# zju-pi/diff-sampler

Hardware: AMD Instinct MI355X
Metric: images/sec (whole node) at NFE=10, EDM CIFAR-10 (higher is better)
Workload: dtype fp32; 1 GPU; EDM CIFAR-10 32x32 SongUNet (55.7M params), DPM-Solver++(2M) logSNR NFE=10, batch 256/GPU; launch=eager

## Files before the change

diff_sampler_amd/csrc/conv3x3_wino.hip:

```cpp
#include <type_traits>

#include "igemm_common.h"

namespace igemm {
namespace {

typedef float f32x2 __attribute__((ext_vector_type(2)));

constexpr int WV_NO_NORM = 2, WV_NO_HALO = 4, WV_NO_DMA = 8, WV_NO_EPI = 16;
constexpr int WINO_K = 8;
constexpr int WINO_POS = 2 * 64 * 4;
constexpr int WINO_IMG = 16 * WINO_POS;
constexpr int WINO_NSH = 4;
constexpr int WINO_EPI_LD = 36;

#define DS_WINO_WAIT_VM0() do { __builtin_amdgcn_s_waitcnt(0x0F70); asm volatile("" ::: "memory"); } while (0)
#define DS_WINO_WAIT_VM(n) do { __builtin_amdgcn_s_waitcnt(0x0F70 | (n)); asm volatile("" ::: "memory"); } while (0)

template <int VAR, int NORM, int NSL>
__global__ void __launch_bounds__(256, 1) conv3x3_wino_kernel(const KParams p) {
    extern __shared__ __attribute__((aligned(16))) float smem[];
    float* Us = smem;
    float* Vs = smem + 2 * WINO_IMG;
    float* Hs = smem + 4 * WINO_IMG;

    const int tid = threadIdx.x, lane = tid & 63;
    const int wave = __builtin_amdgcn_readfirstlane(tid >> 6);
    const int wr = wave >> 1, wc = wave & 1;
    int mt, nt;
    if (!decode_tile(blockIdx.x, p.mtiles, p.ntiles, mt, nt)) return;
    const int m0 = mt * 256, n0 = nt * 64;
    const int img0 = m0 / p.HW;
    const int r0 = (m0 - img0 * p.HW) / p.W;
    const int WPH = p.WP >> 1, Wt = p.W >> 1;
    const int Ctot = p.c0 + p.c1;
    const int nslabs = Ctot / WINO_K;
    constexpr bool kDma = !(VAR & WV_NO_DMA), kHalo = !(VAR & WV_NO_HALO);
    constexpr int kNorm = (VAR & WV_NO_NORM) ? 0 : NORM;

    const int kh_h = tid & 1;
    const int h_buf = p.NP * WINO_K + 4;
    unsigned h_off0[WINO_NSH], h_off1[WINO_NSH];
    int h_lds[WINO_NSH];
#pragma unroll
    for (int j = 0; j < WINO_NSH; ++j) {
        const int hp = (tid + j * 256) >> 1;
        const int hr = hp / p.WP, hc = hp - hr * p.WP;
        const int y = r0 + hr - 1, x = hc - 1;
        const bool in = hp < p.NP;
        const bool ok = in && (unsigned)y < (unsigned)p.H && (unsigned)x < (unsigned)p.W;
        const int pix = min(max(y, 0), p.H - 1) * p.W + min(max(x, 0), p.W - 1);
        h_off0[j] = (unsigned)(pix * p.lda0 + kh_h * 4) * 4u;
        h_off1[j] = (unsigned)(pix * p.lda1 + kh_h * 4) * 4u;
        const int cell = (((kh_h * 2 + (hc & 1)) * p.HP + hr) * WPH + (hc >> 1)) * 4;
        h_lds[j] = ok ? cell : p.NP * WINO_K;
        if (in && !ok) {
            const f32x4 z = {0.f, 0.f, 0.f, 0.f};
            *reinterpret_cast<f32x4*>(Hs + cell) = z;
            *reinterpret_cast<f32x4*>(Hs + h_buf + cell) = z;
        }
    }
    const float* a0i = p.a0 + (size_t)img0 * p.HW * p.lda0;
    const float* a1i = p.a1 + (size_t)img0 * p.HW * p.lda1;
    const float* cpi = p.norm + (size_t)img0 * 3 * Ctot;
    unsigned c_lane = (unsigned)(kh_h * 16);
    struct HaloRegs {
        f32x4 h[WINO_NSH];
        f32x4 mu = {0.f, 0.f, 0.f, 0.f}, ga = {1.f, 1.f, 1.f, 1.f}, be = {0.f, 0.f, 0.f, 0.f};
    };
    HaloRegs hreg;
    float h_t[4 * WINO_NSH], h_u[4 * WINO_NSH];
    const float* h_src = nullptr;
    unsigned h_sel = 0;
    auto halo_src = [&](int s) {
        const int c = s * WINO_K;
        const bool first = c < p.c0;
        h_src = first ? a0i + c : a1i + (c - p.c0);
        h_sel = (unsigned)__builtin_amdgcn_readfirstlane(first ? -1 : 0);
        asm volatile("" : "+s"(h_sel));
    };
    auto halo_load1 = [&](HaloRegs& R, auto J) {
        constexpr int j = decltype(J)::value;
        if constexpr (j >= NSL) return;
        const unsigned off = (h_off0[j] & h_sel) | (h_off1[j] & ~h_sel);
        R.h[j] = *reinterpret_cast<const f32x4*>(reinterpret_cast<const char*>(h_src) + off);
    };
    auto coef_load1 = [&](HaloRegs& R, int s, auto I) {
        constexpr int i = decltype(I)::value;
        if constexpr (NORM != 0) {
            const char* cs = reinterpret_cast<const char*>(cpi + (size_t)i * Ctot + s * WINO_K);
            asm volatile("" : "+v"(c_lane));
            const f32x4 v = *reinterpret_cast<const f32x4*>(cs + c_lane);
            if constexpr (i == 0) R.mu = v; else if constexpr (i == 1) R.ga = v; else R.be = v;
        }
    };
    auto halo_chain = [&](HaloRegs& R, float* hs, auto C, auto ST) {
        constexpr int c = decltype(C)::value, st = decltype(ST)::value, j = c >> 2, e = c & 3;
        if constexpr (j >= NSL) return;
        if constexpr (st == 0 && kNorm != 0) {
            h_t[c] = __builtin_fmaf(R.h[j][e] - R.mu[e], R.ga[e], R.be[e]);
            if constexpr (kNorm == 2) h_u[c] = __expf(-h_t[c]);
        }
        if constexpr (st == 1 && kNorm == 2) h_u[c] = __builtin_amdgcn_rcpf(1.0f + h_u[c]);
        if constexpr (st == 2) {
            float v = R.h[j][e];
            if constexpr (kNorm == 1) v = h_t[c];
            if constexpr (kNorm == 2) v = h_t[c] * h_u[c];
            R.h[j][e] = v;
            if constexpr (e == 3) *reinterpret_cast<f32x4*>(hs + h_lds[j]) = R.h[j];
        }
    };

    const int t_t = (tid >> 1) & 63, cpl = tid & 1, kh_t = tid >> 7;
    const int t_ty = t_t / Wt, t_tx = t_t - t_ty * Wt;
    const int h_rd = ((kh_t * 2 * p.HP + 2 * t_ty) * WPH + t_tx) * 4 + cpl * 2;
    const int h_par = p.HP * WPH * 4;
    const int v_wr = (kh_t * 64 + t_t) * 4 + cpl * 2;
    f32x2 t_d[4][4], t_r[4];
    auto tr_read1 = [&](const float* hs, auto I) {
        constexpr int i = decltype(I)::value >> 2, j = decltype(I)::value & 3;
        t_d[i][j] = *reinterpret_cast<const f32x2*>(hs + h_rd + (j & 1) * h_par + i * WPH * 4 + (j >> 1) * 4);
    };
    auto tr_write1 = [&](float* vs, auto I) {
        constexpr int i = decltype(I)::value >> 2, j = decltype(I)::value & 3;
        if constexpr (j == 0) {
#pragma unroll
            for (int q = 0; q < 4; ++q)
                t_r[q] = i == 0 ? t_d[0][q] - t_d[2][q] : i == 1 ? t_d[1][q] + t_d[2][q] : i == 2 ? t_d[2][q] - t_d[1][q] : t_d[1][q] - t_d[3][q];
        }
        const f32x2 v = j == 0 ? t_r[0] - t_r[2] : j == 1 ? t_r[1] + t_r[2] : j == 2 ? t_r[2] - t_r[1] : t_r[1] - t_r[3];
        *reinterpret_cast<f32x2*>(vs + v_wr + (i * 4 + j) * WINO_POS) = v;
    };

    const float* u_src = p.b + (size_t)nt * nslabs * WINO_IMG;
    unsigned u_lane = (unsigned)tid * 16u;
    auto u_dma1 = [&](const float* src, float* ubuf, auto I) {
        constexpr int i = decltype(I)::value;
        float* dst = ubuf + (i * 256 + wave * 64) * 4;
        typedef const __attribute__((address_space(1))) void* gptr_t;
        typedef __attribute__((address_space(3))) void* lptr_t;
        const char* us = reinterpret_cast<const char*>(src + i * 1024);
        asm volatile("" : "+s"(us));
        asm volatile("" : "+v"(u_lane));
        __builtin_amdgcn_global_load_lds((gptr_t)(us + u_lane), (lptr_t)(dst), 16, 0, 0);
    };

    f32x16 acc[16];
#pragma unroll
    for (int q = 0; q < 16; ++q)
#pragma unroll
        for (int r = 0; r < 16; ++r) acc[q][r] = 0.f;
    const int a_off = ((lane >> 5) * 64 + wr * 32 + (lane & 31)) * 4;
    const int b_off = ((lane >> 5) * 64 + wc * 32 + (lane & 31)) * 4;

#define DS_WINO_I(n) std::integral_constant<int, (n)>{}
#define DS_WINO_EACH4(F) F(0) F(1) F(2) F(3)
#define DS_WINO_EACH16(F, b) F((b) + 0) F((b) + 1) F((b) + 2) F((b) + 3) F((b) + 4) F((b) + 5) F((b) + 6) F((b) + 7)                \
                             F((b) + 8) F((b) + 9) F((b) + 10) F((b) + 11) F((b) + 12) F((b) + 13) F((b) + 14) F((b) + 15)

#define DS_WINO_LOADS(R, sl)                                                                                                           \
    halo_load1(R, DS_WINO_I(0)); halo_load1(R, DS_WINO_I(1)); halo_load1(R, DS_WINO_I(2)); halo_load1(R, DS_WINO_I(3));                \
    coef_load1(R, sl, DS_WINO_I(0)); coef_load1(R, sl, DS_WINO_I(1)); coef_load1(R, sl, DS_WINO_I(2));

    halo_src(0);
    DS_WINO_LOADS(hreg, 0)
    {
        HaloRegs hreg1;
        const int s1 = min(1, nslabs - 1);
        halo_src(s1);
        DS_WINO_LOADS(hreg1, s1)
        DS_RACE_SKEW(wave);
#define DS_WINO_F(i) u_dma1(u_src, Us, DS_WINO_I(i)); u_dma1(u_src, Us, DS_WINO_I((i) + 4));
        DS_WINO_EACH4(DS_WINO_F)
#undef DS_WINO_F
        DS_RACE_SKEW(wave);
#define DS_WINO_CHAIN1(c) halo_chain(hreg, Hs, DS_WINO_I(c), DS_WINO_I(0)); halo_chain(hreg, Hs, DS_WINO_I(c), DS_WINO_I(1));          \
                          halo_chain(hreg, Hs, DS_WINO_I(c), DS_WINO_I(2));
        DS_WINO_EACH16(DS_WINO_CHAIN1, 0)
#undef DS_WINO_CHAIN1
        DS_RACE_SKEW(wave);
#define DS_WINO_CHAIN1(c) halo_chain(hreg1, Hs + h_buf, DS_WINO_I(c), DS_WINO_I(0)); halo_chain(hreg1, Hs + h_buf, DS_WINO_I(c), DS_WINO_I(1)); \
                          halo_chain(hreg1, Hs + h_buf, DS_WINO_I(c), DS_WINO_I(2));
        DS_WINO_EACH16(DS_WINO_CHAIN1, 0)
#undef DS_WINO_CHAIN1
    }
    {
        const int s2 = min(2, nslabs - 1);
        halo_src(s2);
        DS_WINO_LOADS(hreg, s2)
    }
    __syncthreads();
#define DS_WINO_F(i) tr_read1(Hs, DS_WINO_I(i));
    DS_WINO_EACH16(DS_WINO_F, 0)
#undef DS_WINO_F
    DS_RACE_SKEW(wave);
#define DS_WINO_F(i) tr_write1(Vs, DS_WINO_I(i));
    DS_WINO_EACH16(DS_WINO_F, 0)
#undef DS_WINO_F
    DS_WINO_WAIT_VM0();
    __syncthreads();

    f32x4 fa[2][4], fb[2][4];
    int s = 0;
    do {
        const int par = s & 1;
        const float* ub = Us + par * WINO_IMG;
        const float* vb = Vs + par * WINO_IMG;
        float* ubn = Us + (par ^ 1) * WINO_IMG;
        float* vbn = Vs + (par ^ 1) * WINO_IMG;
        float* hb = Hs + par * h_buf;
        const float* hbn = Hs + (par ^ 1) * h_buf;
        const int s1 = min(s + 1, nslabs - 1), s3 = min(s + 3, nslabs - 1);
        const float* un = u_src + (size_t)s1 * WINO_IMG;
        auto frag_read = [&](auto G, auto I) {
            constexpr int g = decltype(G)::value, i = decltype(I)::value;
            if constexpr (i < 4) fa[g & 1][i] = *reinterpret_cast<const f32x4*>(vb + (g * 4 + i) * WINO_POS + a_off);
            else fb[g & 1][i - 4] = *reinterpret_cast<const f32x4*>(ub + (g * 4 + i - 4) * WINO_POS + b_off);
        };
#define DS_WINO_F(i) tr_read1(hbn, DS_WINO_I(i));
        DS_WINO_EACH16(DS_WINO_F, 0)
#undef DS_WINO_F
        if constexpr (kHalo) {
            DS_RACE_SKEW(wave);
#define DS_WINO_CHAIN1(c) halo_chain(hreg, hb, DS_WINO_I(c), DS_WINO_I(0)); halo_chain(hreg, hb, DS_WINO_I(c), DS_WINO_I(1));          \
                          halo_chain(hreg, hb, DS_WINO_I(c), DS_WINO_I(2));
            DS_WINO_EACH16(DS_WINO_CHAIN1, 0)
#undef DS_WINO_CHAIN1
            halo_src(s3);
        }
        DS_RACE_SKEW(wave);
#define DS_WINO_F(i) tr_write1(vbn, DS_WINO_I(i));
        DS_WINO_EACH16(DS_WINO_F, 0)
#undef DS_WINO_F
        auto fill = [&](auto K) {
            constexpr int k = decltype(K)::value, g = k >> 4;
            if constexpr (k < 8) {
                if constexpr (kDma) {
                    if constexpr (k == 0) DS_RACE_SKEW(wave);
                    u_dma1(un, ubn, DS_WINO_I(k));
                }
            } else if constexpr (k < 12) {
                if constexpr (kHalo) halo_load1(hreg, DS_WINO_I(k - 8));
            } else if constexpr (k < 15) {
                if constexpr (kHalo) coef_load1(hreg, s3, DS_WINO_I(k - 12));
            }
            constexpr int fr = g == 0 ? 8 : g == 1 ? 20 : g == 2 ? 32 : 64;
            if constexpr (k >= fr && k < fr + 8) frag_read(DS_WINO_I(g + 1), DS_WINO_I(k - fr));
        };
#define DS_WINO_STEP(k)                                                                                                                \
        acc[((k) >> 4) * 4 + ((k) & 3)] = __builtin_amdgcn_mfma_f32_32x32x2f32(fa[((k) >> 4) & 1][(k) & 3][((k) >> 2) & 3],            \
                                                                               fb[((k) >> 4) & 1][(k) & 3][((k) >> 2) & 3],            \
                                                                               acc[((k) >> 4) * 4 + ((k) & 3)], 0, 0, 0);              \
        fill(DS_WINO_I(k));                                                                                                            \
        __builtin_amdgcn_sched_barrier(0);
#define DS_WINO_F(i) frag_read(DS_WINO_I(0), DS_WINO_I(i)); frag_read(DS_WINO_I(0), DS_WINO_I((i) + 4));
        DS_WINO_EACH4(DS_WINO_F)
#undef DS_WINO_F
        __builtin_amdgcn_sched_barrier(0);
        DS_WINO_EACH16(DS_WINO_STEP, 0)
        DS_WINO_EACH16(DS_WINO_STEP, 16)
        DS_WINO_EACH16(DS_WINO_STEP, 32)
        DS_WINO_EACH16(DS_WINO_STEP, 48)
#undef DS_WINO_STEP
        DS_WINO_WAIT_VM0();
        __syncthreads();
    } while (++s < nslabs);
#undef DS_WINO_LOADS

    if constexpr ((VAR & WV_NO_EPI) != 0) {
#pragma unroll
        for (int q = 0; q < 16; ++q) asm volatile("" :: "v"(acc[q]));
        return;
    }

    f32x16 Y[4];
#pragma unroll
    for (int a = 0; a < 2; ++a) {
        f32x16 t[4];
#pragma unroll
        for (int j = 0; j < 4; ++j) t[j] = a == 0 ? acc[j] + acc[4 + j] + acc[8 + j] : acc[4 + j] - acc[8 + j] - acc[12 + j];
        Y[a * 2 + 0] = t[0] + t[1] + t[2];
        Y[a * 2 + 1] = t[1] - t[2] - t[3];
    }

    const int nextra = (p.ec0 + p.ec1) / 32;
    if (nextra > 0) {
        const float* wsk = p.b + (size_t)p.ntiles * nslabs * WINO_IMG + (size_t)nt * nextra * 2048 + tid * 4;
        const int e_chunk = tid & 7;
        int e_lds[8];
#pragma unroll
        for (int j = 0; j < 8; ++j) {
            const int lp = (tid >> 3) + 32 * j;
            const int yl = lp / p.W, x = lp - yl * p.W;
            const int ph = (yl & 1) * 2 + (x & 1), t = (yl >> 1) * Wt + (x >> 1);
            e_lds[j] = (((ph * 4 + (e_chunk >> 1)) * 2 + (e_chunk & 1)) * 64 + (t ^ e_chunk)) * 4;
        }
        int ea_off[4];
#pragma unroll
        for (int g = 0; g < 4; ++g) ea_off[g] = ((lane >> 5) * 64 + ((wr * 32 + (lane & 31)) ^ (2 * g + (lane >> 5)))) * 4;
        const unsigned e_t0 = (unsigned)((tid >> 3) * p.elda0 + e_chunk * 4), e_t1 = (unsigned)((tid >> 3) * p.elda1 + e_chunk * 4);
        const float* e_src = nullptr;
        unsigned e_off = 0;
        int e_step = 0;
        auto e_sel = [&](int es) {
            const int c = es * 32;
            const bool first = c < p.ec0;
            const int ld = first ? p.elda0 : p.elda1;
            e_src = (first ? p.e0 + c : p.e1 + (c - p.ec0)) + (size_t)m0 * ld;
            e_step = 32 * ld;
            e_off = first ? e_t0 : e_t1;
        };
        auto e_load1 = [&](f32x4* dst, auto J) {
            constexpr int j = decltype(J)::value;
            dst[j] = *reinterpret_cast<const f32x4*>(e_src + (size_t)(j * e_step) + e_off);
        };
        auto w_dma1 = [&](int es, float* wbuf, auto I) {
            constexpr int i = decltype(I)::value;
            float* dst = wbuf + (i * 256 + wave * 64) * 4;
            typedef const __attribute__((address_space(1))) void* gptr_t;
            typedef __attribute__((address_space(3))) void* lptr_t;
            __builtin_amdgcn_global_load_lds((gptr_t)(wsk + (size_t)es * 2048 + i * 1024), (lptr_t)(dst), 16, 0, 0);
        };
#define DS_WINO_EACH8(F) F(0) F(1) F(2) F(3) F(4) F(5) F(6) F(7)

        f32x4 ereg[8];
        {
            f32x4 ereg0[8];
            DS_RACE_SKEW(wave);
            w_dma1(0, smem, DS_WINO_I(0)); w_dma1(0, smem, DS_WINO_I(1));
            e_sel(0);
#define DS_WINO_F(j) e_load1(ereg0, DS_WINO_I(j));
            DS_WINO_EACH8(DS_WINO_F)
#undef DS_WINO_F
            e_sel(min(1, nextra - 1));
#define DS_WINO_F(j) e_load1(ereg, DS_WINO_I(j));
            DS_WINO_EACH8(DS_WINO_F)
#undef DS_WINO_F
            DS_WINO_WAIT_VM(8);
            DS_RACE_SKEW(wave);
#pragma unroll
            for (int j = 0; j < 8; ++j) *reinterpret_cast<f32x4*>(Vs + e_lds[j]) = ereg0[j];
        }
        __syncthreads();

        f32x4 ga[2][4], gb[2];
        int es = 0;
        do {
            const float* vb = smem + (2 - (es & 1)) * WINO_IMG;
            float* vn = smem + (1 + (es & 1)) * WINO_IMG;
            const float* wb = smem + (es & 1) * 2048;
            float* wn = smem + ((es + 1) & 1) * 2048;
            const int es1 = min(es + 1, nextra - 1);
            e_sel(min(es + 2, nextra - 1));
            auto frag_read = [&](auto G, auto I) {
                constexpr int g = decltype(G)::value, i = decltype(I)::value;
                if constexpr (i < 4) ga[g & 1][i] = *reinterpret_cast<const f32x4*>(vb + (i * 4 + g) * WINO_POS + ea_off[g]);
                else gb[g & 1] = *reinterpret_cast<const f32x4*>(wb + g * WINO_POS + b_off);
            };
            auto fill = [&](auto K) {
                constexpr int k = decltype(K)::value, g = k >> 4;
                if constexpr (k < 2) {
                    if constexpr (k == 0) DS_RACE_SKEW(wave);
                    w_dma1(es1, wn, DS_WINO_I(k));
                } else if constexpr (k >= 7 && k < 15) {
                    if constexpr (k == 7) DS_RACE_SKEW(wave);
                    *reinterpret_cast<f32x4*>(vn + e_lds[k - 7]) = ereg[k - 7];
                } else if constexpr (k >= 15 && k < 23) {
                    e_load1(ereg, DS_WINO_I(k - 15));
                }
                constexpr int fr = g == 0 ? 2 : g == 1 ? 24 : g == 2 ? 36 : 64;
                if constexpr (k >= fr && k < fr + 5) frag_read(DS_WINO_I(g + 1), DS_WINO_I(k - fr));
            };
#define DS_WINO_STEP(k)                                                                                                                \
            Y[(k) & 3] = __builtin_amdgcn_mfma_f32_32x32x2f32(ga[((k) >> 4) & 1][(k) & 3][((k) >> 2) & 3], gb[((k) >> 4) & 1][((k) >> 2) & 3], \
                                                              Y[(k) & 3], 0, 0, 0);                                                    \
            fill(DS_WINO_I(k));                                                                                                        \
            __builtin_amdgcn_sched_barrier(0);
            frag_read(DS_WINO_I(0), DS_WINO_I(0)); frag_read(DS_WINO_I(0), DS_WINO_I(4)); frag_read(DS_WINO_I(0), DS_WINO_I(1));
            frag_read(DS_WINO_I(0), DS_WINO_I(2)); frag_read(DS_WINO_I(0), DS_WINO_I(3));
            __builtin_amdgcn_sched_barrier(0);
            DS_WINO_EACH16(DS_WINO_STEP, 0)
            DS_WINO_EACH16(DS_WINO_STEP, 16)
            DS_WINO_EACH16(DS_WINO_STEP, 32)
            DS_WINO_EACH16(DS_WINO_STEP, 48)
#undef DS_WINO_STEP
            DS_WINO_WAIT_VM0();
            __syncthreads();
        } while (++es < nextra);
#undef DS_WINO_EACH8
    }
#undef DS_WINO_EACH16
#undef DS_WINO_EACH4
#undef DS_WINO_I

    float* stage = smem + wave * 32 * WINO_EPI_LD;
    const int c4 = (lane & 7) * 4;
    const int col = n0 + wc * 32 + c4;
    f32x4 cb = {0.f, 0.f, 0.f, 0.f}, cvu = {0.f, 0.f, 0.f, 0.f};
    if (p.colbias) cb = *reinterpret_cast<const f32x4*>(p.colbias + col);
    if (p.cbias) cvu = *reinterpret_cast<const f32x4*>(p.cbias + (size_t)(p.cbias_bcast ? 0 : img0) * p.cbias_ld + col);
    const float acc_scale = __builtin_bit_cast(float, __builtin_amdgcn_readfirstlane(__builtin_bit_cast(int, p.acc_scale)));
    const float scale = __builtin_bit_cast(float, __builtin_amdgcn_readfirstlane(__builtin_bit_cast(int, p.scale)));
    int e_row[4];
#pragma unroll
    for (int pass = 0; pass < 4; ++pass) {
        const int tl = wr * 32 + pass * 8 + (lane >> 3);
        const int ty = tl / Wt, tx = tl - ty * Wt;
        e_row[pass] = m0 + 2 * ty * p.W + 2 * tx;
    }
#pragma unroll
    for (int a = 0; a < 2; ++a) {
        f32x4 st_s = {0.f, 0.f, 0.f, 0.f}, st_q = {0.f, 0.f, 0.f, 0.f};
#pragma unroll
        for (int b = 0; b < 2; ++b) {
            const f32x16 y = Y[a * 2 + b];
            f32x4 rv[4];
            if (p.res) {
#pragma unroll
                for (int pass = 0; pass < 4; ++pass)
                    rv[pass] = __builtin_nontemporal_load(reinterpret_cast<const f32x4*>(p.res + (size_t)(e_row[pass] + a * p.W + b) * p.res_ld + col));
            }
#pragma unroll
            for (int r = 0; r < 16; ++r) stage[((r & 3) + 8 * (r >> 2) + 4 * (lane >> 5)) * WINO_EPI_LD + (lane & 31)] = y[r];
#pragma unroll
            for (int pass = 0; pass < 4; ++pass) {
                f32x4 v = *reinterpret_cast<const f32x4*>(stage + (pass * 8 + (lane >> 3)) * WINO_EPI_LD + c4);
                v *= acc_scale;
                v += cb;
                if (p.cbias) v += cvu;
                if (p.res) v += rv[pass];
                v *= scale;
                if (p.act == DS_ACT_SILU) {
#pragma unroll
                    for (int q = 0; q < 4; ++q) v[q] = ds_silu(v[q]);
                }
                __builtin_nontemporal_store(v, reinterpret_cast<f32x4*>(p.out + (size_t)(e_row[pass] + a * p.W + b) * p.ldo + col));
                st_s += v; st_q += v * v;
            }
        }
        if (p.stats) {
#pragma unroll
            for (int q = 0; q < 4; ++q) {
                st_s[q] += __shfl_xor(st_s[q], 8); st_s[q] += __shfl_xor(st_s[q], 16); st_s[q] += __shfl_xor(st_s[q], 32);
                st_q[q] += __shfl_xor(st_q[q], 8); st_q[q] += __shfl_xor(st_q[q], 16); st_q[q] += __shfl_xor(st_q[q], 32);
            }
            if (lane < 8) {
                float* sp = p.stats + (size_t)((m0 >> 6) + wr * 2 + a) * 2 * p.N + col;
                *reinterpret_cast<f32x4*>(sp) = st_s;
                *reinterpret_cast<f32x4*>(sp + p.N) = st_q;
            }
        }
    }
}

template <int VAR, int NORM, int NSL>
int launch_wino_ns(KParams& p, hipStream_t stream) {
    const int smem = (4 * WINO_IMG + 2 * (p.NP * WINO_K + 4)) * (int)sizeof(float);
    DS_ENSURE_DYN_LDS((&conv3x3_wino_kernel<VAR, NORM, NSL>), 160 * 1024);
    hipLaunchKernelGGL((conv3x3_wino_kernel<VAR, NORM, NSL>), dim3(grid_1d(p.mtiles, p.ntiles)), dim3(256), smem, stream, p);
    DS_CHECK_LAUNCH();
    return DS_OK;
}

template <int VAR, int NORM>
int launch_wino_n(KParams& p, hipStream_t stream) {
    return p.NP * 2 <= 3 * 256 ? launch_wino_ns<VAR, NORM, 3>(p, stream) : launch_wino_ns<VAR, NORM, 4>(p, stream);
}

template <int VAR>
int launch_wino(KParams& p, hipStream_t stream) {
    if (!p.norm) return launch_wino_n<VAR, 0>(p, stream);
    return p.norm_act == DS_ACT_SILU ? launch_wino_n<VAR, 2>(p, stream) : launch_wino_n<VAR, 1>(p, stream);
}

}

bool conv3x3_wino_applicable(const KParams& p) {
    if (p.taps != 9 || p.stride != 1 || p.splits != 1 || (p.ec0 & 31) || (p.ec1 & 31)) return false;
    if ((p.H & 1) || (p.W & 1) || p.W < 4 || p.W > 64 || p.HW % 256 || 256 % p.W || ((256 / p.W) & 1)) return false;
    if ((p.N & 63) || (p.c0 % WINO_K) || (p.c1 % WINO_K) || !p.vec_ok || p.out_planar || p.out_f16 || p.res_f16 || p.rowbias) return false;
    if (p.act != DS_ACT_NONE && p.act != DS_ACT_SILU) return false;
    const int np = (256 / p.W + 2) * (p.W + 2);
    if (np * 2 > WINO_NSH * 256 || (4 * WINO_IMG + 2 * (np * WINO_K + 4)) * (int)sizeof(float) > 160 * 1024) return false;
    return p.M % 256 == 0;
}

int launch_conv3x3_wino(KParams& p, hipStream_t stream) {
    if (!conv3x3_wino_applicable(p)) return DS_E_SHAPE;
    p.TH = 256 / p.W; p.nimg = 1; p.HP = p.TH + 2; p.WP = p.W + 2; p.NP = p.HP * p.WP;
    p.mtiles = p.M / 256; p.ntiles = p.N / 64; p.n_begin = 0;
#ifdef DS_CONV_ABLATIONS
    if (p.t_variant & 0x10000) {
        switch (p.t_variant & 31) {
            case 2: return launch_wino<2>(p, stream);
            case 4: return launch_wino<4>(p, stream);
            case 8: return launch_wino<8>(p, stream);
            case 16: return launch_wino<16>(p, stream);
            case 28: return launch_wino<28>(p, stream);
            default: break;
        }
    }
#endif
    return launch_wino<0>(p, stream);
}

}
```

Measured before the change: 471.3 images/sec.

## Add 128x128-tile Winograd conv3x3 kernel for channel counts divisible by 128

Adds a new Winograd 3x3 convolution kernel that tiles 128 output pixels by 128 output channels instead of 256x64, with its own halo staging, input-transform layout, MFMA pipeline, skip-connection GEMM and epilogue. Dispatch sends all shapes with N divisible by 128 to the new kernel unless a variant bit disables it. The squarer tile is meant to improve operand reuse and halve LDS use, allowing better balance on wider-channel layers. The cost is fewer pixel rows per tile, so a larger share of loaded rows are halo, and a lot of new hand-scheduled code that could regress on some shapes.

```diff
diff --git a/diff_sampler_amd/csrc/conv3x3_wino.hip b/diff_sampler_amd/csrc/conv3x3_wino.hip
--- a/diff_sampler_amd/csrc/conv3x3_wino.hip
+++ b/diff_sampler_amd/csrc/conv3x3_wino.hip
@@ -453,6 +453,446 @@
     }
 }
 
+constexpr int WN_POS = 2 * 32 * 4;
+constexpr int WN_IMG = 16 * WN_POS;
+constexpr int WN_NSH = 3;
+
+template <int NORM, int NSL>
+__global__ void __launch_bounds__(256, 1) wino_n128_kernel(const KParams p) {
+    extern __shared__ __attribute__((aligned(16))) float smem[];
+    float* Vs = smem;
+    float* Hs = smem + 2 * WN_IMG;
+
+    const int tid = threadIdx.x, lane = tid & 63;
+    const int wave = __builtin_amdgcn_readfirstlane(tid >> 6);
+    int mt, nt;
+    if (!decode_tile(blockIdx.x, p.mtiles, p.ntiles, mt, nt)) return;
+    const int m0 = mt * 128, n0 = nt * 128;
+    const int img0 = m0 / p.HW;
+    const int r0 = (m0 - img0 * p.HW) / p.W;
+    const int WPH = p.WP >> 1, Wt = p.W >> 1;
+    const int Ctot = p.c0 + p.c1;
+    const int nslabs = Ctot / WINO_K;
+
+    const int kh_h = tid & 1;
+    const int h_buf = p.NP * WINO_K + 4;
+    unsigned h_off0[WN_NSH], h_off1[WN_NSH];
+    int h_lds[WN_NSH];
+#pragma unroll
+    for (int j = 0; j < WN_NSH; ++j) {
+        const int hp = (tid + j * 256) >> 1;
+        const int hr = hp / p.WP, hc = hp - hr * p.WP;
+        const int y = r0 + hr - 1, x = hc - 1;
+        const bool in = hp < p.NP;
+        const bool ok = in && (unsigned)y < (unsigned)p.H && (unsigned)x < (unsigned)p.W;
+        const int pix = min(max(y, 0), p.H - 1) * p.W + min(max(x, 0), p.W - 1);
+        h_off0[j] = (unsigned)(pix * p.lda0 + kh_h * 4) * 4u;
+        h_off1[j] = (unsigned)(pix * p.lda1 + kh_h * 4) * 4u;
+        const int cell = (((kh_h * 2 + (hc & 1)) * p.HP + hr) * WPH + (hc >> 1)) * 4;
+        h_lds[j] = ok ? cell : p.NP * WINO_K;
+        if (in && !ok) {
+            const f32x4 z = {0.f, 0.f, 0.f, 0.f};
+            *reinterpret_cast<f32x4*>(Hs + cell) = z;
+            *reinterpret_cast<f32x4*>(Hs + h_buf + cell) = z;
+        }
+    }
+    const float* a0i = p.a0 + (size_t)img0 * p.HW * p.lda0;
+    const float* a1i = p.a1 + (size_t)img0 * p.HW * p.lda1;
+    const float* cpi = p.norm + (size_t)img0 * 3 * Ctot;
+    unsigned c_lane = (unsigned)(kh_h * 16);
+    struct HaloRegs {
+        f32x4 h[WN_NSH];
+        f32x4 mu = {0.f, 0.f, 0.f, 0.f}, ga = {1.f, 1.f, 1.f, 1.f}, be = {0.f, 0.f, 0.f, 0.f};
+    };
+    HaloRegs hreg;
+    float h_t[4 * WN_NSH], h_u[4 * WN_NSH];
+    const float* h_src = nullptr;
+    unsigned h_sel = 0;
+    auto halo_src = [&](int s) {
+        const int c = s * WINO_K;
+        const bool first = c < p.c0;
+        h_src = first ? a0i + c : a1i + (c - p.c0);
+        h_sel = (unsigned)__builtin_amdgcn_readfirstlane(first ? -1 : 0);
+        asm volatile("" : "+s"(h_sel));
+    };
+    auto halo_load1 = [&](HaloRegs& R, auto J) {
+        constexpr int j = decltype(J)::value;
+        if constexpr (j < NSL) {
+            const unsigned off = (h_off0[j] & h_sel) | (h_off1[j] & ~h_sel);
+            R.h[j] = *reinterpret_cast<const f32x4*>(reinterpret_cast<const char*>(h_src) + off);
+        }
+    };
+    auto coef_load1 = [&](HaloRegs& R, int s, auto I) {
+        constexpr int i = decltype(I)::value;
+        if constexpr (NORM != 0) {
+            const char* cs = reinterpret_cast<const char*>(cpi + (size_t)i * Ctot + s * WINO_K);
+            asm volatile("" : "+v"(c_lane));
+            const f32x4 v = *reinterpret_cast<const f32x4*>(cs + c_lane);
+            if constexpr (i == 0) R.mu = v; else if constexpr (i == 1) R.ga = v; else R.be = v;
+        }
+    };
+    auto halo_chain = [&](HaloRegs& R, float* hs, auto C, auto ST) {
+        constexpr int c = decltype(C)::value, st = decltype(ST)::value, j = c >> 2, e = c & 3;
+        if constexpr (j < NSL) {
+            if constexpr (st == 0 && NORM != 0) {
+                h_t[c] = __builtin_fmaf(R.h[j][e] - R.mu[e], R.ga[e], R.be[e]);
+                if constexpr (NORM == 2) h_u[c] = __expf(-h_t[c]);
+            }
+            if constexpr (st == 1 && NORM == 2) h_u[c] = __builtin_amdgcn_rcpf(1.0f + h_u[c]);
+            if constexpr (st == 2) {
+                float v = R.h[j][e];
+                if constexpr (NORM == 1) v = h_t[c];
+                if constexpr (NORM == 2) v = h_t[c] * h_u[c];
+                R.h[j][e] = v;
+                if constexpr (e == 3) *reinterpret_cast<f32x4*>(hs + h_lds[j]) = R.h[j];
+            }
+        }
+    };
+
+    const int t_t = (tid >> 1) & 31, cpl = tid & 1, kh_t = wave & 1, half = wave >> 1;
+    const int t_ty = t_t / Wt, t_tx = t_t - t_ty * Wt;
+    const int h_rd = ((kh_t * 2 * p.HP + 2 * t_ty + half) * WPH + t_tx) * 4 + cpl * 2;
+    const int h_par = p.HP * WPH * 4;
+    const int v_wr = (kh_t * 32 + t_t) * 4 + cpl * 2 + half * 8 * WN_POS;
+    f32x2 t_e[3][4];
+    auto tr_read1 = [&](const float* hs, auto I) {
+        constexpr int i = decltype(I)::value >> 2, j = decltype(I)::value & 3;
+        t_e[i][j] = *reinterpret_cast<const f32x2*>(hs + h_rd + (j & 1) * h_par + i * WPH * 4 + (j >> 1) * 4);
+    };
+    auto tr_write = [&](float* vs) {
+        f32x2 ra[4], rb[4];
+        if (half == 0) {
+#pragma unroll
+            for (int q = 0; q < 4; ++q) { ra[q] = t_e[0][q] - t_e[2][q]; rb[q] = t_e[1][q] + t_e[2][q]; }
+        } else {
+#pragma unroll
+            for (int q = 0; q < 4; ++q) { ra[q] = t_e[1][q] - t_e[0][q]; rb[q] = t_e[0][q] - t_e[2][q]; }
+        }
+#pragma unroll
+        for (int i = 0; i < 2; ++i) {
+            const f32x2* t_r = i == 0 ? ra : rb;
+#pragma unroll
+            for (int j = 0; j < 4; ++j) {
+                const f32x2 v = j == 0 ? t_r[0] - t_r[2] : j == 1 ? t_r[1] + t_r[2] : j == 2 ? t_r[2] - t_r[1] : t_r[1] - t_r[3];
+                *reinterpret_cast<f32x2*>(vs + v_wr + (i * 4 + j) * WN_POS) = v;
+            }
+        }
+    };
+
+    const float* u_src = p.b + (size_t)(2 * nt + (wave >> 1)) * nslabs * WINO_IMG;
+    unsigned b_lane = (unsigned)(((lane >> 5) * 64 + (wave & 1) * 32 + (lane & 31)) * 16);
+    f32x4 fa[2][4], fb[2][4];
+    typedef const __attribute__((address_space(1))) f32x4* gf4_t;
+    auto b_load1 = [&](const float* src, auto G, auto I) {
+        constexpr int g = decltype(G)::value, i = decltype(I)::value;
+        const char* us = reinterpret_cast<const char*>(src + (g * 4 + i) * WINO_POS);
+        asm volatile("" : "+s"(us));
+        asm volatile("" : "+v"(b_lane));
+        fb[g & 1][i] = *(gf4_t)(us + b_lane);
+    };
+
+    f32x16 acc[16];
+#pragma unroll
+    for (int q = 0; q < 16; ++q)
+#pragma unroll
+        for (int r = 0; r < 16; ++r) acc[q][r] = 0.f;
+    const int a_off = ((lane >> 5) * 32 + (lane & 31)) * 4;
+
+#define DS_WINO_I(n) std::integral_constant<int, (n)>{}
+#define DS_WINO_EACH4(F) F(0) F(1) F(2) F(3)
+#define DS_WINO_EACH12(F) F(0) F(1) F(2) F(3) F(4) F(5) F(6) F(7) F(8) F(9) F(10) F(11)
+#define DS_WINO_EACH16(F, b) F((b) + 0) F((b) + 1) F((b) + 2) F((b) + 3) F((b) + 4) F((b) + 5) F((b) + 6) F((b) + 7)                \
+                             F((b) + 8) F((b) + 9) F((b) + 10) F((b) + 11) F((b) + 12) F((b) + 13) F((b) + 14) F((b) + 15)
+#define DS_WINO_LOADS(R, sl)                                                                                                           \
+    halo_load1(R, DS_WINO_I(0)); halo_load1(R, DS_WINO_I(1)); halo_load1(R, DS_WINO_I(2));                                             \
+    coef_load1(R, sl, DS_WINO_I(0)); coef_load1(R, sl, DS_WINO_I(1)); coef_load1(R, sl, DS_WINO_I(2));
+
+    halo_src(0);
+    DS_WINO_LOADS(hreg, 0)
+    {
+        HaloRegs hreg1;
+        const int s1 = min(1, nslabs - 1);
+        halo_src(s1);
+        DS_WINO_LOADS(hreg1, s1)
+#define DS_WINO_F(i) b_load1(u_src, DS_WINO_I(0), DS_WINO_I(i));
+        DS_WINO_EACH4(DS_WINO_F)
+#undef DS_WINO_F
+        DS_RACE_SKEW(wave);
+#define DS_WINO_CHAIN1(c) halo_chain(hreg, Hs, DS_WINO_I(c), DS_WINO_I(0)); halo_chain(hreg, Hs, DS_WINO_I(c), DS_WINO_I(1));          \
+                          halo_chain(hreg, Hs, DS_WINO_I(c), DS_WINO_I(2));
+        DS_WINO_EACH12(DS_WINO_CHAIN1)
+#undef DS_WINO_CHAIN1
+        DS_RACE_SKEW(wave);
+#define DS_WINO_CHAIN1(c) halo_chain(hreg1, Hs + h_buf, DS_WINO_I(c), DS_WINO_I(0)); halo_chain(hreg1, Hs + h_buf, DS_WINO_I(c), DS_WINO_I(1)); \
+                          halo_chain(hreg1, Hs + h_buf, DS_WINO_I(c), DS_WINO_I(2));
+        DS_WINO_EACH12(DS_WINO_CHAIN1)
+#undef DS_WINO_CHAIN1
+    }
+    {
+        const int s2 = min(2, nslabs - 1);
+        halo_src(s2);
+        DS_WINO_LOADS(hreg, s2)
+    }
+    __syncthreads();
+#define DS_WINO_TR1(i) tr_read1(Hs, DS_WINO_I(i));
+    DS_WINO_EACH12(DS_WINO_TR1)
+#undef DS_WINO_TR1
+    DS_RACE_SKEW(wave);
+    tr_write(Vs);
+    DS_WINO_WAIT_VM0();
+    __syncthreads();
+
+    int s = 0;
+    do {
+        const int par = s & 1;
+        const float* vb = Vs + par * WN_IMG;
+        float* vbn = Vs + (par ^ 1) * WN_IMG;
+        float* hb = Hs + par * h_buf;
+        const float* hbn = Hs + (par ^ 1) * h_buf;
+        const int s1 = min(s + 1, nslabs - 1), s3 = min(s + 3, nslabs - 1);
+        const float* uc = u_src + (size_t)s * WINO_IMG;
+        const float* un = u_src + (size_t)s1 * WINO_IMG;
+        auto a_read = [&](auto G, auto I) {
+            constexpr int g = decltype(G)::value, i = decltype(I)::value;
+            fa[g & 1][i] = *reinterpret_cast<const f32x4*>(vb + (g * 4 + i) * WN_POS + a_off);
+        };
+#define DS_WINO_TR1(i) tr_read1(hbn, DS_WINO_I(i));
+        DS_WINO_EACH12(DS_WINO_TR1)
+#undef DS_WINO_TR1
+        DS_RACE_SKEW(wave);
+#define DS_WINO_CHAIN1(c) halo_chain(hreg, hb, DS_WINO_I(c), DS_WINO_I(0)); halo_chain(hreg, hb, DS_WINO_I(c), DS_WINO_I(1));          \
+                          halo_chain(hreg, hb, DS_WINO_I(c), DS_WINO_I(2));
+        DS_WINO_EACH12(DS_WINO_CHAIN1)
+#undef DS_WINO_CHAIN1
+        halo_src(s3);
+        DS_RACE_SKEW(wave);
+        tr_write(vbn);
+        auto fill = [&](auto K) {
+            constexpr int k = decltype(K)::value, g = k >> 4, q = k & 15;
+            if constexpr (q < 4) {
+                if constexpr (g < 3) b_load1(uc, DS_WINO_I(g + 1), DS_WINO_I(q));
+                else b_load1(un, DS_WINO_I(0), DS_WINO_I(q));
+            } else if constexpr (k < 7) {
+                halo_load1(hreg, DS_WINO_I(k - 4));
+            } else if constexpr (k < 10) {
+                coef_load1(hreg, s3, DS_WINO_I(k - 7));
+            } else if constexpr (q >= 10 && q < 14 && g < 3) {
+                a_read(DS_WINO_I(g + 1), DS_WINO_I(q - 10));
+            }
+        };
+#define DS_WINO_STEP(k)                                                                                                                \
+        acc[((k) >> 4) * 4 + ((k) & 3)] = __builtin_amdgcn_mfma_f32_32x32x2f32(fa[((k) >> 4) & 1][(k) & 3][((k) >> 2) & 3],            \
+                                                                               fb[((k) >> 4) & 1][(k) & 3][((k) >> 2) & 3],            \
+                                                                               acc[((k) >> 4) * 4 + ((k) & 3)], 0, 0, 0);              \
+        fill(DS_WINO_I(k));                                                                                                            \
+        __builtin_amdgcn_sched_barrier(0);
+#define DS_WINO_F(i) a_read(DS_WINO_I(0), DS_WINO_I(i));
+        DS_WINO_EACH4(DS_WINO_F)
+#undef DS_WINO_F
+        __builtin_amdgcn_sched_barrier(0);
+        DS_WINO_EACH16(DS_WINO_STEP, 0)
+        DS_WINO_EACH16(DS_WINO_STEP, 16)
+        DS_WINO_EACH16(DS_WINO_STEP, 32)
+        DS_WINO_EACH16(DS_WINO_STEP, 48)
+#undef DS_WINO_STEP
+        __syncthreads();
+    } while (++s < nslabs);
+#undef DS_WINO_LOADS
+
+    f32x16 Y[4];
+#pragma unroll
+    for (int a = 0; a < 2; ++a) {
+        f32x16 t[4];
+#pragma unroll
+        for (int j = 0; j < 4; ++j) t[j] = a == 0 ? acc[j] + acc[4 + j] + acc[8 + j] : acc[4 + j] - acc[8 + j] - acc[12 + j];
+        Y[a * 2 + 0] = t[0] + t[1] + t[2];
+        Y[a * 2 + 1] = t[1] - t[2] - t[3];
+    }
+
+    const int nextra = (p.ec0 + p.ec1) / 32;
+    if (nextra > 0) {
+        const float* wsk = p.b + (size_t)(p.N / 64) * nslabs * WINO_IMG + (size_t)(2 * nt + (wave >> 1)) * nextra * 2048;
+        const int e_chunk = tid & 7;
+        int e_lds[4];
+#pragma unroll
+        for (int j = 0; j < 4; ++j) {
+            const int lp = (tid >> 3) + 32 * j;
+            const int yl = lp / p.W, x = lp - yl * p.W;
+            const int ph = (yl & 1) * 2 + (x & 1), t = (yl >> 1) * Wt + (x >> 1);
+            e_lds[j] = (((ph * 4 + (e_chunk >> 1)) * 2 + (e_chunk & 1)) * 32 + (t ^ e_chunk)) * 4;
+        }
+        int ea_off[4];
+#pragma unroll
+        for (int g = 0; g < 4; ++g) ea_off[g] = ((lane >> 5) * 32 + ((lane & 31) ^ (2 * g + (lane >> 5)))) * 4;
+        const unsigned e_t0 = (unsigned)((tid >> 3) * p.elda0 + e_chunk * 4), e_t1 = (unsigned)((tid >> 3) * p.elda1 + e_chunk * 4);
+        const float* e_src = nullptr;
+        unsigned e_off = 0;
+        int e_step = 0;
+        auto e_sel = [&](int es) {
+            const int c = es * 32;
+            const bool first = c < p.ec0;
+            const int ld = first ? p.elda0 : p.elda1;
+            e_src = (first ? p.e0 + c : p.e1 + (c - p.ec0)) + (size_t)m0 * ld;
+            e_step = 32 * ld;
+            e_off = first ? e_t0 : e_t1;
+        };
+        auto e_load1 = [&](f32x4* dst, auto J) {
+            constexpr int j = decltype(J)::value;
+            dst[j] = *reinterpret_cast<const f32x4*>(e_src + (size_t)(j * e_step) + e_off);
+        };
+        f32x4 ga[2][4], gb[2];
+        auto w_load1 = [&](int es, auto G) {
+            constexpr int g = decltype(G)::value;
+            const char* ws = reinterpret_cast<const char*>(wsk + (size_t)es * 2048 + g * WINO_POS);
+            asm volatile("" : "+s"(ws));
+            asm volatile("" : "+v"(b_lane));
+            gb[g & 1] = *(gf4_t)(ws + b_lane);
+        };
+
+        f32x4 ereg[4];
+        {
+            f32x4 ereg0[4];
+            w_load1(0, DS_WINO_I(0));
+            e_sel(0);
+#define DS_WINO_F(j) e_load1(ereg0, DS_WINO_I(j));
+            DS_WINO_EACH4(DS_WINO_F)
+#undef DS_WINO_F
+            e_sel(min(1, nextra - 1));
+#define DS_WINO_F(j) e_load1(ereg, DS_WINO_I(j));
+            DS_WINO_EACH4(DS_WINO_F)
+#undef DS_WINO_F
+            DS_RACE_SKEW(wave);
+#pragma unroll
+            for (int j = 0; j < 4; ++j) *reinterpret_cast<f32x4*>(Vs + e_lds[j]) = ereg0[j];
+        }
+        __syncthreads();
+
+        int es = 0;
+        do {
+            const float* vb = smem + (es & 1) * WN_IMG;
+            float* vn = smem + ((es + 1) & 1) * WN_IMG;
+            const int es1 = min(es + 1, nextra - 1);
+            e_sel(min(es + 2, nextra - 1));
+            auto a_read = [&](auto G, auto I) {
+                constexpr int g = decltype(G)::value, i = decltype(I)::value;
+                ga[g & 1][i] = *reinterpret_cast<const f32x4*>(vb + (i * 4 + g) * WN_POS + ea_off[g]);
+            };
+            auto fill = [&](auto K) {
+                constexpr int k = decltype(K)::value, g = k >> 4, q = k & 15;
+                if constexpr (q == 0) {
+                    if constexpr (g < 3) w_load1(es, DS_WINO_I(g + 1));
+                    else w_load1(es1, DS_WINO_I(0));
+                } else if constexpr (q < 5) {
+                    if constexpr (g < 3) a_read(DS_WINO_I(g + 1), DS_WINO_I(q - 1));
+                } else if constexpr (k < 9) {
+                    if constexpr (k == 5) DS_RACE_SKEW(wave);
+                    *reinterpret_cast<f32x4*>(vn + e_lds[k - 5]) = ereg[k - 5];
+                } else if constexpr (k < 13) {
+                    e_load1(ereg, DS_WINO_I(k - 9));
+                }
+            };
+#define DS_WINO_STEP(k)                                                                                                                \
+            Y[(k) & 3] = __builtin_amdgcn_mfma_f32_32x32x2f32(ga[((k) >> 4) & 1][(k) & 3][((k) >> 2) & 3], gb[((k) >> 4) & 1][((k) >> 2) & 3], \
+                                                              Y[(k) & 3], 0, 0, 0);                                                    \
+            fill(DS_WINO_I(k));                                                                                                        \
+            __builtin_amdgcn_sched_barrier(0);
+#define DS_WINO_F(i) a_read(DS_WINO_I(0), DS_WINO_I(i));
+            DS_WINO_EACH4(DS_WINO_F)
+#undef DS_WINO_F
+            __builtin_amdgcn_sched_barrier(0);
+            DS_WINO_EACH16(DS_WINO_STEP, 0)
+            DS_WINO_EACH16(DS_WINO_STEP, 16)
+            DS_WINO_EACH16(DS_WINO_STEP, 32)
+            DS_WINO_EACH16(DS_WINO_STEP, 48)
+#undef DS_WINO_STEP
+            __syncthreads();
+        } while (++es < nextra);
+    }
+#undef DS_WINO_EACH16
+#undef DS_WINO_EACH12
+#undef DS_WINO_EACH4
+#undef DS_WINO_I
+
+    float* stage = smem + wave * 32 * WINO_EPI_LD;
+    const int c4 = (lane & 7) * 4;
+    const int col = n0 + wave * 32 + c4;
+    f32x4 cb = {0.f, 0.f, 0.f, 0.f}, cvu = {0.f, 0.f, 0.f, 0.f};
+    if (p.colbias) cb = *reinterpret_cast<const f32x4*>(p.colbias + col);
+    if (p.cbias) cvu = *reinterpret_cast<const f32x4*>(p.cbias + (size_t)(p.cbias_bcast ? 0 : img0) * p.cbias_ld + col);
+    const float acc_scale = __builtin_bit_cast(float, __builtin_amdgcn_readfirstlane(__builtin_bit_cast(int, p.acc_scale)));
+    const float scale = __builtin_bit_cast(float, __builtin_amdgcn_readfirstlane(__builtin_bit_cast(int, p.scale)));
+    int e_row[4];
+#pragma unroll
+    for (int pass = 0; pass < 4; ++pass) {
+        const int tl = pass * 8 + (lane >> 3);
+        const int ty = tl / Wt, tx = tl - ty * Wt;
+        e_row[pass] = m0 + 2 * ty * p.W + 2 * tx;
+    }
+#pragma unroll
+    for (int a = 0; a < 2; ++a) {
+        f32x4 st_s = {0.f, 0.f, 0.f, 0.f}, st_q = {0.f, 0.f, 0.f, 0.f};
+#pragma unroll
+        for (int b = 0; b < 2; ++b) {
+            const f32x16 y = Y[a * 2 + b];
+            f32x4 rv[4];
+            if (p.res) {
+#pragma unroll
+                for (int pass = 0; pass < 4; ++pass)
+                    rv[pass] = __builtin_nontemporal_load(reinterpret_cast<const f32x4*>(p.res + (size_t)(e_row[pass] + a * p.W + b) * p.res_ld + col));
+            }
+#pragma unroll
+            for (int r = 0; r < 16; ++r) stage[((r & 3) + 8 * (r >> 2) + 4 * (lane >> 5)) * WINO_EPI_LD + (lane & 31)] = y[r];
+#pragma unroll
+            for (int pass = 0; pass < 4; ++pass) {
+                f32x4 v = *reinterpret_cast<const f32x4*>(stage + (pass * 8 + (lane >> 3)) * WINO_EPI_LD + c4);
+                v *= acc_scale;
+                v += cb;
+                if (p.cbias) v += cvu;
+                if (p.res) v += rv[pass];
+                v *= scale;
+                if (p.act == DS_ACT_SILU) {
+#pragma unroll
+                    for (int q = 0; q < 4; ++q) v[q] = ds_silu(v[q]);
+                }
+                __builtin_nontemporal_store(v, reinterpret_cast<f32x4*>(p.out + (size_t)(e_row[pass] + a * p.W + b) * p.ldo + col));
+                st_s += v; st_q += v * v;
+            }
+        }
+        if (p.stats) {
+#pragma unroll
+            for (int q = 0; q < 4; ++q) {
+                st_s[q] += __shfl_xor(st_s[q], 8); st_s[q] += __shfl_xor(st_s[q], 16); st_s[q] += __shfl_xor(st_s[q], 32);
+                st_q[q] += __shfl_xor(st_q[q], 8); st_q[q] += __shfl_xor(st_q[q], 16); st_q[q] += __shfl_xor(st_q[q], 32);
+            }
+            if (lane < 8) {
+                float* sp = p.stats + (size_t)((m0 >> 6) + a) * 2 * p.N + col;
+                *reinterpret_cast<f32x4*>(sp) = st_s;
+                *reinterpret_cast<f32x4*>(sp + p.N) = st_q;
+            }
+        }
+    }
+}
+
+template <int NORM, int NSL>
+int launch_wino_n128_ns(KParams& p, hipStream_t stream) {
+    const int smem = (2 * WN_IMG + 2 * (p.NP * WINO_K + 4)) * (int)sizeof(float);
+    DS_ENSURE_DYN_LDS((&wino_n128_kernel<NORM, NSL>), 64 * 1024);
+    hipLaunchKernelGGL((wino_n128_kernel<NORM, NSL>), dim3(grid_1d(p.mtiles, p.ntiles)), dim3(256), smem, stream, p);
+    DS_CHECK_LAUNCH();
+    return DS_OK;
+}
+
+template <int NORM>
+int launch_wino_n128_n(KParams& p, hipStream_t stream) {
+    return p.NP * 2 <= 2 * 256 ? launch_wino_n128_ns<NORM, 2>(p, stream) : launch_wino_n128_ns<NORM, 3>(p, stream);
+}
+
+int launch_wino_n128(KParams& p, hipStream_t stream) {
+    if (!p.norm) return launch_wino_n128_n<0>(p, stream);
+    return p.norm_act == DS_ACT_SILU ? launch_wino_n128_n<2>(p, stream) : launch_wino_n128_n<1>(p, stream);
+}
+
+
 template <int VAR, int NORM, int NSL>
 int launch_wino_ns(KParams& p, hipStream_t stream) {
     const int smem = (4 * WINO_IMG + 2 * (p.NP * WINO_K + 4)) * (int)sizeof(float);
@@ -501,6 +941,11 @@
         }
     }
 #endif
+    if (!(p.t_variant & 1024) && p.N % 128 == 0) {
+        p.TH = 128 / p.W; p.HP = p.TH + 2; p.NP = p.HP * p.WP;
+        p.mtiles = p.M / 128; p.ntiles = p.N / 128;
+        return launch_wino_n128(p, stream);
+    }
     return launch_wino<0>(p, stream);
 }
 
```

Result: faster. 492.5 images/sec, median of 6 (+4.5%).
